# ben-watt-es/madigan

Hardware: AMD Instinct MI355X
Metric: env-steps/sec (batched) at 8192 envs × 8 assets; % HBM roofline (higher is better)
Workload: dtype f64; 1 GPU; C3: TrendOU x8 assets per env, slippage 1e-4 + 2% cost broker, DDR eta=.001 n=1, discrete actions via action_to_transaction, auto-reset; nstep=1, n_envs_per_gpu=8192, n_envs_total=8192, n_assets=8, window=0, assets_per_lane=1, schedule=trio, parallelism=env-sharded x1 (no per-step collective)

## Files before the change

### madigan_amd/csrc/mgn_diag.h

```cpp
#pragma once

#if !defined(MGN_DIAG) &&                                                                            \
    (defined(MGN_STAMPS) || defined(MGN_WALLX) || defined(MGN_ITERSTAMP) || defined(MGN_ABL_NOSTORE) ||  \
     defined(MGN_ABL_NOSTORE_ASSET) || defined(MGN_ABL_NOSTORE_ENV) || defined(MGN_ABL_DRAW) ||          \
     defined(MGN_TRIO_ABL_PRO) || defined(MGN_TRIO_ABL_G) || defined(MGN_TRIO_ABL_L) ||                  \
     defined(MGN_TRIO_ABL_F) || defined(MGN_TRIO_ABL_EPI) || defined(MGN_NST_ABL_TERM) ||                \
     defined(MGN_NST_ABL_SUM) || defined(MGN_NST_ABL_ROW) || defined(MGN_NO_GK) ||                      \
     defined(MGN_ABL_PLAIN_OFF))
#error "stamp / ablation switches belong to diagnostic builds (-DMGN_DIAG, tools/build_variant.py)"
#endif

namespace mgn {

#ifdef MGN_STAMPS
#define MGN_ST(...) __VA_ARGS__
#else
#define MGN_ST(...)
#endif
#ifdef MGN_TRIO_ABL_PRO
constexpr bool kAblPro = true;
#else
constexpr bool kAblPro = false;
#endif
#ifdef MGN_TRIO_ABL_G
// ... 39 lines not shown
#ifdef MGN_ABL_NOSTORE_ENV
constexpr bool kAblNoStoreEnv = true;
#else
constexpr bool kAblNoStoreEnv = false;
#endif
#ifdef MGN_ABL_PLAIN_OFF
constexpr bool kAblPlainOff = true;
#else
constexpr bool kAblPlainOff = false;
#endif

#ifdef MGN_STAMPS
__device__ unsigned long long g_duo_stamps[24];
__device__ unsigned long long g_trio_par[16];
#define MGN_PAR(acc, j, work, wait)                      \
  {                                                      \
    const unsigned long long w_ = (work), a_ = (wait);   \
    const bool o_ = ((j) & 1) != 0;                      \
    acc[0] += o_ ? 0 : w_;                               \
    acc[1] += o_ ? 0 : a_;                               \
    acc[2] += o_ ? w_ : 0;                               \
    acc[3] += o_ ? a_ : 0;                               \
  }
__shared__ unsigned long long s_duo_sub[8];
__device__ unsigned long long g_duo_wall[2048 * 32];
#define MGN_T(v) v = __builtin_amdgcn_s_memtime()
#define MGN_WALL(i) if ((threadIdx.x & 255) == 0 && blockIdx.x < 2048) g_duo_wall[blockIdx.x * 32 + (i)] = __builtin_amdgcn_s_memrealtime()
#elif defined(MGN_WALLX)
__device__ unsigned long long g_duo_stamps[24];
__device__ unsigned long long g_duo_wall[2048 * 32];
#define MGN_T(v)
#define MGN_WALL(i) if ((threadIdx.x & 255) == 0 && blockIdx.x < 2048) g_duo_wall[blockIdx.x * 32 + (i)] = __builtin_amdgcn_s_memrealtime()
#else
#define MGN_T(v)
#define MGN_WALL(i)
#endif
#ifdef MGN_WALLX
#define MGN_RT(v) v = __builtin_amdgcn_s_memrealtime()
#define MGN_WALLV(i, val_) if ((threadIdx.x & 255) == 0 && blockIdx.x < 2048) g_duo_wall[blockIdx.x * 32 + (i)] = (val_)
#else
#define MGN_RT(v)
#define MGN_WALLV(i, val_)
#endif

#ifdef MGN_ITERSTAMP
__device__ unsigned long long g_iter[256 * 64];
// ... 12 lines not shown
```

### madigan_amd/csrc/mgn_launch_a8t.hip

```cpp
#include "mgn_launch_impl.h"
MGN_DEFINE_UNIT(a8t)
#if defined(MGN_STAMPS) || defined(MGN_WALLX)
extern "C" int mgn_diag_stamps(unsigned long long* h) {
  if (hipMemcpyFromSymbol(h, HIP_SYMBOL(mgn::g_duo_stamps), 24 * sizeof(unsigned long long)) != hipSuccess)
    return 1;
  unsigned long long z[24] = {};
  return hipMemcpyToSymbol(HIP_SYMBOL(mgn::g_duo_stamps), z, sizeof(z)) != hipSuccess;
}
#ifdef MGN_STAMPS
extern "C" int mgn_diag_parity(unsigned long long* h) {
  if (hipMemcpyFromSymbol(h, HIP_SYMBOL(mgn::g_trio_par), 16 * sizeof(unsigned long long)) != hipSuccess)
    return 1;
  unsigned long long z[16] = {};
  return hipMemcpyToSymbol(HIP_SYMBOL(mgn::g_trio_par), z, sizeof(z)) != hipSuccess;
}
#endif
extern "C" int mgn_diag_wall(unsigned long long* h) {
  return hipMemcpyFromSymbol(h, HIP_SYMBOL(mgn::g_duo_wall), 2048 * 32 * sizeof(unsigned long long)) != hipSuccess;
}
#endif
#ifdef MGN_ITERSTAMP
extern "C" int mgn_diag_iter(unsigned long long* h) {
  if (hipMemcpyFromSymbol(h, HIP_SYMBOL(mgn::g_iter), 256 * 64 * sizeof(unsigned long long)) != hipSuccess)
    return 1;
  static unsigned long long z[256 * 64] = {};
  return hipMemcpyToSymbol(HIP_SYMBOL(mgn::g_iter), z, sizeof(z)) != hipSuccess;
}
#endif
```

### madigan_amd/csrc/mgn_math.h

```cpp
#pragma once

#include <hip/hip_runtime.h>
#include <stdint.h>

namespace mgn {

__device__ __forceinline__ double bits_to_d(uint64_t u) { return __longlong_as_double((long long)u); }
__device__ __forceinline__ uint64_t d_to_bits(double d) { return (uint64_t)__double_as_longlong(d); }

struct u4 { uint32_t x, y, z, w; };

__device__ __forceinline__ u4 philox4x32_10(uint32_t c0, uint32_t c1, uint32_t c2, uint32_t c3,
                                            uint32_t k0, uint32_t k1) {
#pragma unroll
  for (int r = 0; r < 10; ++r) {
    const uint64_t p0 = (uint64_t)0xD2511F53u * c0;
    const uint64_t p1 = (uint64_t)0xCD9E8D57u * c2;
    const uint32_t n0 = (uint32_t)(p1 >> 32) ^ c1 ^ k0;
    const uint32_t n2 = (uint32_t)(p0 >> 32) ^ c3 ^ k1;
    c0 = n0; c1 = (uint32_t)p1; c2 = n2; c3 = (uint32_t)p0;
    k0 += 0x9E3779B9u;
    k1 += 0xBB67AE85u;
  }
  return u4{c0, c1, c2, c3};
// ... 126 lines not shown
  q = __builtin_fma(__builtin_fma(-y, q, x), r, q);
  if (!fast) {
    double xs = x;
    asm volatile("" : "+v"(xs));
    q = xs / y;
  }
  return q;
}
__device__ __forceinline__ double rt_div(double a, double b) {
  if (!__builtin_amdgcn_class(b, kNormalClass)) return a / b;
  double r = __builtin_amdgcn_rcp(b);
  r = __builtin_fma(r, __builtin_fma(-b, r, 1.0), r);
  r = __builtin_fma(r, __builtin_fma(-b, r, 1.0), r);
  return a * r;
}
__device__ __forceinline__ double rt_sqrt(double x) {
  if (!__builtin_amdgcn_class(x, 1 << 8)) return sqrt(x);
  const double y = __builtin_amdgcn_rsq(x);
  double g = x * y, h = 0.5 * y;
  const double r = __builtin_fma(-g, h, 0.5);
  g = __builtin_fma(g, r, g);
  h = __builtin_fma(h, r, h);
  return __builtin_fma(__builtin_fma(-g, g, x), h, g);
}

struct Draw {
  double z, ut;
  uint32_t dbit;
};

__device__ __forceinline__ double v_log(double x) {
  const double ln2_hi = bits_to_d(0x3fe62e42fee00000ull);
  const double ln2_lo = bits_to_d(0x3dea39ef35793c76ull);
  const double Lg1 = bits_to_d(0x3FE5555555555593ull), Lg2 = bits_to_d(0x3FD999999997FA04ull),
               Lg3 = bits_to_d(0x3FD2492494229359ull), Lg4 = bits_to_d(0x3FCC71C51D8E78AFull),
               Lg5 = bits_to_d(0x3FC7466496CB03DEull), Lg6 = bits_to_d(0x3FC39A09D078C69Full),
               Lg7 = bits_to_d(0x3FC2F112DF3E5244ull);
  const uint64_t ix = d_to_bits(x);
  int32_t hx = (int32_t)(ix >> 32);
  int32_t k = ((hx >> 20) & 0x7ff) - 1023;
  hx &= 0x000fffff;
  const int32_t i = (hx + 0x95f64) & 0x100000;
  k += (i >> 20);
  const uint64_t mb = ((uint64_t)(uint32_t)(hx | (i ^ 0x3ff00000)) << 32) | (ix & 0xffffffffull);
  const double f = bits_to_d(mb) - 1.0;
  const double s = f / (2.0 + f);
// ... 81 lines not shown
__device__ __forceinline__ double normal_of(const u4& x) {
  double sn, cs;
  v_sincos2pi((double)x.z * TWO_M32, sn, cs);
  return v_radius(x) * cs;
}

__device__ __forceinline__ double log_ratio(double x) {
  const double d = x - 1.0;
  if (fabs(d) <= 0.03125) {
    const double u = x + 1.0;
    const double e = x - (u - 1.0);
    const double sh = rt_div(d, u);
    const double r = __fma_rn(-sh, u, d);
    const double sl = (r - sh * e) * 0.5;
    const double s2 = sh * sh;
    const double t =
        s2 * (0.3333333333333333 + s2 * (0.2 + s2 * (0.14285714285714285 + s2 * 0.1111111111111111)));
    const double s_2 = sh + sh;
    return s_2 + ((sl + sl) + s_2 * t);
  }
  return log(x);
}

__device__ __forceinline__ double frac_part(double x) { return copysign(x - trunc(x), x); }

__device__ __forceinline__ double log_norm(double x) { return log((x < 1e-5) ? 1e-5 : x); }

__device__ __noinline__ double det_asin(double x) {
  const double pio2_hi = bits_to_d(0x3FF921FB54442D18ull), pio2_lo = bits_to_d(0x3C91A62633145C07ull),
               pio4_hi = bits_to_d(0x3FE921FB54442D18ull);
  const double pS0 = bits_to_d(0x3FC5555555555555ull), pS1 = bits_to_d(0xBFD4D61203EB6F7Dull),
               pS2 = bits_to_d(0x3FC9C1550E884455ull), pS3 = bits_to_d(0xBFA48228B5688F3Bull),
               pS4 = bits_to_d(0x3F49EFE07501B288ull), pS5 = bits_to_d(0x3F023DE10DFDF709ull),
               qS1 = bits_to_d(0xC0033A271C8A2D4Bull), qS2 = bits_to_d(0x40002AE59C598AC8ull),
               qS3 = bits_to_d(0xBFE6066C1B8D0159ull), qS4 = bits_to_d(0x3FB3B8C5B12E9282ull);
  const uint64_t bx = d_to_bits(x);
  const int32_t hx = (int32_t)(bx >> 32);
  const int32_t ix = hx & 0x7fffffff;
  if (ix >= 0x3ff00000) {
    if (((ix - 0x3ff00000) | (int32_t)(uint32_t)bx) == 0) return x * pio2_hi + x * pio2_lo;
    return (x - x) / (x - x);
  }
  if (ix < 0x3fe00000) {
    if (ix < 0x3e400000) return x;
    const double t = x * x;
    const double p = t * (pS0 + t * (pS1 + t * (pS2 + t * (pS3 + t * (pS4 + t * pS5)))));
// ... 25 lines not shown
```

### madigan_amd/csrc/mgn_shapers.h

```cpp
#pragma once

#include <hip/hip_runtime.h>
#include <stdint.h>

#include "../../include/madigan_amd.h"
#include "mgn_math.h"
#include "mgn_params.h"
#include "mgn_reduce.h"

namespace mgn {

__device__ __forceinline__ double dsr_one(double r, double A, double B) {
  const double dA = r - A;
  const double dB = r * r - B;
  const double t = B - A * A;
  const double a = fabs(t);
  return rt_div(B * dA - (A * dB) / 2, a * rt_sqrt(a) + 1.1920928955078125e-07);
}
__device__ __forceinline__ double ddr_one(double r, double A, double B) {
  const double sB = rt_sqrt(B);
  const double h = r - A / 2;
  const bool pos = r > 0.;
  const double num = pos ? h : (B * h - (A * (r * r)) / 2);
  const double den = (pos ? sB : B * sB) + 1.1920928955078125e-07;
  return rt_div(num, den);
}
struct DdrPre {
  double hA, dpos, dneg;
};
__device__ __forceinline__ DdrPre ddr_pre(double A, double B) {
  const double sB = rt_sqrt(B);
  return DdrPre{A / 2, sB + 1.1920928955078125e-07, B * sB + 1.1920928955078125e-07};
}
__device__ __forceinline__ double ddr_one_pre(double r, double A, double B, const DdrPre& q) {
  const double h = r - q.hA;
  const bool pos = r > 0.;
  const double num = pos ? h : (B * h - (A * (r * r)) / 2);
  return rt_div(num, pos ? q.dpos : q.dneg);
}
__device__ __forceinline__ double rt_rcp(double b) {
  double r = __builtin_amdgcn_rcp(b);
  r = __builtin_fma(r, __builtin_fma(-b, r, 1.0), r);
  return __builtin_fma(r, __builtin_fma(-b, r, 1.0), r);
}
__device__ __forceinline__ double div_pre(double a, double b, double rb) {
  double q = a * rb;
  if (!__builtin_amdgcn_class(b, kNormalClass)) {
    double x = a;
    asm volatile("" : "+v"(x));
    q = x / b;
  }
  return q;
}
struct DdrPreR {
  DdrPre q;
  double rpos, rneg;
};
__device__ __forceinline__ DdrPreR ddr_pre_r(double A, double B) {
  const DdrPre q = ddr_pre(A, B);
  return DdrPreR{q, rt_rcp(q.dpos), rt_rcp(q.dneg)};
}
// ... 271 lines not shown
```

### madigan_amd/csrc/mgn_trio.h

```cpp
#pragma once

#include <hip/hip_runtime.h>
#include <stdint.h>

#include "../../include/madigan_amd.h"
#include "mgn_broker.h"
#include "mgn_consts.h"
#include "mgn_diag.h"
#include "mgn_gout.h"
#include "mgn_lane.h"
#include "mgn_math.h"
#include "mgn_params.h"
#include "mgn_reduce.h"
#include "mgn_rows.h"
#include "mgn_select.h"
#include "mgn_shapers.h"
#include "mgn_sources.h"

namespace mgn {


constexpr int kPrioG = 0, kPrioL = 2, kPrioF = 1;

constexpr int kNstU = 3;


__device__ __forceinline__ bool trio_exit(int j, int K, const int32_t& more) {
  if (j < K) return false;
  return !__builtin_amdgcn_readfirstlane(more);
}

template <int M, int S, bool ONE>
__device__ __forceinline__ bool rec_done(const double (&Lr)[M], const double (&P)[M], double cashv, double ml,
                                         double shv, double b, bool any_mc, const KParams& p, Sums& q,
                                         double& curEq) {
  double tlp[M];
#pragma unroll
  for (int m = 0; m < M; ++m) tlp[m] = Lr[m] * P[m];
  q.lp = canon<M, S, ONE>(tlp);
  q.ml = ml;
  q.sh = shv;
  q.b = b;
  curEq = (cashv + q.lp) - q.b;
  return any_mc || margin_call(q, cashv, p.mainM) || (curEq < 0.1 * p.init_cash);
}
// ... 66 lines not shown
  warm_kernargs<(int)(48 + sizeof(KParams) + sizeof(mgn_traj) + 8 + 16 + 4)>();
  MGN_IT(47, 0);
  const int in_kind = DISC ? IN_DISCRETE : in_kind_rt;
  constexpr int M = MM;
  constexpr bool TAIL = K1 && !RP && !WIN && MM == 1;
  constexpr bool GLOG = WIN && !RP;
  constexpr int NPADS = 2;
  constexpr bool NRUN = NST == 2;
  constexpr bool SBR = NRUN && TW == 64;
  static_assert(M == 1 || (M == 2 && !NST), "two slots per lane: one-step rewards");
  static_assert(!ONE || (S == 2 && M == 1), "a one-asset env on two lanes per role");
  constexpr int APAD = S * M;
  constexpr int TRIO_W = TW;
  constexpr int TRIO_BLOCK = 3 * TW;
  constexpr int EPB = TRIO_W / S;
  __shared__ TrioShared<S, TW, M> sh;
  __shared__ EnvRecs<APAD> recs[EPB];
  __shared__ mgn_asset_source s_src[APAD];
  __shared__ double s_tgt[MGN_MAX_ASSETS + 1];
  __shared__ double s_disc[NST ? MGN_MAX_NSTEP : 1];
  __shared__ double s_disc2[SBR ? MGN_MAX_NSTEP : 1];
  extern __shared__ __attribute__((aligned(16))) double s_nst[];
  constexpr bool FB = S == 8 && MM == 1 && !WIN && !NST && !RP && !ONE && !K1;
  __shared__ __attribute__((aligned(16))) double s_fqc[FB ? TW : 1], s_fqp[FB ? TW : 1], s_fqx[FB ? TW : 1],
      s_fqr[FB ? TW : 1];
  __shared__ int32_t s_fqk[FB ? TW : 1];
  const int role = threadIdx.x / TRIO_W;
  const int l = threadIdx.x % TRIO_W;
  constexpr bool GSLOT = GK < 0 && !RP && TW / S > 1 && M == 1;
  constexpr bool TAIL_EXACT = TAIL && !GSLOT;
  const int el = (GSLOT && role == 0) ? l % EPB : l / S;
  const int ls = (GSLOT && role == 0) ? l / EPB : l % S;
  const int lx = (el * S + ls) * M;
  const int env = blockIdx.x * EPB + el;
  const bool live = env < p.N;
  const int envc = live ? env : 0;
  const int A = p.A;
  Lane<M> s;
#pragma unroll
  for (int m = 0; m < M; ++m) {
    s.asset[m] = ls * M + m;
    s.valid[m] = live && ls * M + m < A;
  }
  s.rcur = 0;
  s.row = 0;
  s.pf_ok = false;
  s.fcol = (RP && p.F <= APAD) ? ls * M : -1;
  const size_t li = (size_t)envc * A + (s.valid[0] ? ls * M : 0);
  constexpr int NQ = (RP || M > 1) ? 0 : GK == MGN_SRC_TRENDOU ? 9 : GK == MGN_SRC_OU ? 3 : 0;
  constexpr bool QREG = NQ > 0;
  double qr[QREG ? NQ : 1];
  const double* const tgt_g = p.target;
#pragma unroll
  for (int m = 0; m < M; ++m) {
    s.P[m] = kAblPro ? 5.0 : ((s.valid[m] && role != 2) ? kP[li + m] : 0.);
    s.L[m] = s.mep[m] = s.Bm[m] = s.sx[m] = s.oum[m] = s.dy[m] = 0.;
    s.tlen[m] = 0;
    s.tfl[m] = 0;
  }
  uint64_t ts = 0;
  double cash = 0.;
  int act_cur[M] = {};
  const MGN_G int8_t* act_lane = vptr(act_in) + li;
  double ep_ret = 0., ep_len = 0., n_done = 0.;
  double shA = 0., shB = 0.;
  int32_t rhead = 0, rlen = 0;
  int32_t nlen = 0, nhead = 0;
  NstRun nrs{0., 0., 0., 0., 0., 0.};
  int32_t nsl = 0;
  int32_t fcnt = 0, fdone = 0;
  if (!kAblPro && role == 0) {
    constexpr bool r_sx = GK < 0 || GK == MGN_SRC_SINE || GK == MGN_SRC_SAWTOOTH || GK == MGN_SRC_TRIANGLE ||
                          GK == MGN_SRC_TRENDYOU;
    constexpr bool r_oum = GK < 0 || GK == MGN_SRC_TRENDOU || GK == MGN_SRC_TRENDYOU || GK == MGN_SRC_OUPAIR;
    constexpr bool r_trend = GK < 0 || GK == MGN_SRC_TRENDOU || GK == MGN_SRC_SIMPLETREND ||
                             GK == MGN_SRC_TRENDYOU;
#pragma unroll
    for (int m = 0; m < M; ++m) {
      if (s.valid[m]) {
        if (r_sx) s.sx[m] = p.sx[li + m];
        if (r_oum) s.oum[m] = p.oum[li + m];
        if (r_trend) {
          s.dy[m] = p.dy[li + m];
          s.tlen[m] = p.tlen[li + m];
          s.tfl[m] = p.tfl[li + m];
        }
      }
    }
    if constexpr (QREG) {
      const double* q = p.src[s.valid[0] ? ls : 0].p;
#pragma unroll
      for (int i = 0; i < NQ; ++i) qr[i] = q[i];
    }
// ... 143 lines not shown
  if (role == 0) {
    p.seed = in_vgpr(p.seed);
    p.env_offset = in_vgpr(p.env_offset);
    drain_vmem();
    MGN_IT(54, 0);
    int k = 0;
    constexpr bool SV_P = GK < 0 || !(GK == MGN_SRC_TRENDOU || GK == MGN_SRC_SIMPLETREND ||
                                      GK == MGN_SRC_TRENDYOU || GK == MGN_SRC_OUPAIR);
    constexpr bool SV_SX = GK < 0 || GK != MGN_SRC_TRENDYOU;
    constexpr bool SV_OUM = GK < 0 || !(GK == MGN_SRC_TRENDOU || GK == MGN_SRC_TRENDYOU || GK == MGN_SRC_OUPAIR);
    constexpr bool SV_TLEN = GK < 0 || !(GK == MGN_SRC_TRENDOU || GK == MGN_SRC_SIMPLETREND || GK == MGN_SRC_TRENDYOU);
    constexpr bool SV_TFL = GK < 0 || GK != MGN_SRC_SIMPLETREND;
    double svP[M] = {}, svSx[M] = {}, svOum[M] = {}, svDy[M] = {};
    int32_t svTlen[M] = {};
    uint8_t svTfl[M] = {};
    uint64_t svTs = 0;
    Lane<M> s2;
    gen_state_copy<M>(s2, s);
    uint64_t ts2 = 0;
    bool shadow = false, tail_it = false, stored = false;
    int jlast = 0;
    __builtin_amdgcn_s_setprio(kPrioG);
    MGN_ST(unsigned long long T0 = 0, T1 = 0, T2 = 0, acc0 = 0, acc1 = 0, par[4] = {0, 0, 0, 0},
           dev[4] = {0, 0, 0, 0}; int jn = 0;)
    int gpend = 0;
    RpCurM<M> rp{};
    RpNextM<M> rnx{};
    auto tick = [&]() {
      if constexpr (RP) {
        trio_replay_tick<M>(s, p, ts, rp, rnx);
      } else {
        gen_tick<M, false, false, GK, true, (M > 1)>(s, p, env, ts, QREG ? qr : nullptr);
        ts = ts + 1;
      }
    };
    auto g_store = [&]() {
#pragma unroll
      for (int m = 0; m < M; ++m) {
        const int kd = GK >= 0 ? GK : s.kind[m];
        const bool w_sx =
            kd == MGN_SRC_SINE || kd == MGN_SRC_SAWTOOTH || kd == MGN_SRC_TRIANGLE || kd == MGN_SRC_TRENDYOU;
        const bool w_oum = kd == MGN_SRC_TRENDOU || kd == MGN_SRC_TRENDYOU || kd == MGN_SRC_OUPAIR;
        const bool w_trend = kd == MGN_SRC_TRENDOU || kd == MGN_SRC_SIMPLETREND || kd == MGN_SRC_TRENDYOU;
        if (s.valid[m]) {
          const size_t i = (size_t)env * A + s.asset[m];
          p.P[i] = s.P[m];
          if (w_sx) p.sx[i] = s.sx[m];
// ... 105 lines not shown
        sh.price[cur][lx + m] = s.P[m];
        if (DISC) sh.prcp[cur][lx + m] = rcp_refined(s.P[m]);
      }
      if constexpr (GLOG) {
        if (p.ring_log != 0) {
#pragma unroll
          for (int m = 0; m < M; ++m) sh.lprice[cur][lx + m] = log_norm(s.P[m]);
        }
      }
      if (ls == 0) sh.ts[cur][el] = ts;
      if constexpr (RP) {
        if (ls == 0) {
          sh.row[cur][el] = rp.row;
          sh.dend[cur][el] = rp.dend;
        }
#pragma unroll
        for (int m = 0; m < M; ++m) sh.feat[cur][lx + m] = rp.curF[m];
      }
      if (j == 0) MGN_IT(48, 0);
      MGN_T(T1);
      __syncthreads();
      MGN_T(T2);
      MGN_IT(2 + (j < 40 ? j : 40), 0);
      MGN_ST(acc0 += T1 - T0; acc1 += T2 - T1; jn = j; MGN_PAR(par, j, T1 - T0, T2 - T1))
      jlast = j;
      if (trio_exit(j, K, sh.more[j % 3])) break;
    }
    MGN_ST(if (threadIdx.x == 0) {
      atomicAdd(&g_duo_stamps[0], acc0);
      atomicAdd(&g_duo_stamps[1], acc1);
      atomicAdd(&g_duo_stamps[8], (unsigned long long)(jn + 1));
      atomicAdd(&g_duo_stamps[10], 1ull);
      for (int i = 0; i < 4; ++i) atomicAdd(&g_trio_par[i], par[i]);
      atomicAdd(&g_trio_par[12], dev[0]);
      atomicAdd(&g_trio_par[13], dev[2]);
      atomicAdd(&g_trio_par[14], dev[1]);
      atomicAdd(&g_trio_par[15], dev[3]);
    })
    if constexpr (kAblEpi) return;
    if constexpr (TAIL) {
      if (live && shadow && !sh.reset[jlast & 1][el]) {
        gen_state_copy<M>(s, s2);
        ts = ts2;
      }
    }
    if (live && !stored) {
      g_store();
      if (RP && ls == 0) p.rcur[env] = s.rcur;
    }
    MGN_IT_DRAIN();
    MGN_IT(44, 0);
    return;
  }

  if (role == 1) {
    const uint32_t om = OMC ? OMC : traj_mask(out);
    const MGN_G double* gunits = vptr(units_in);
    const MGN_G int32_t* gaidx = vptr(aidx_in);
    p.init_cash = in_vgpr(p.init_cash);
    p.mainM = in_vgpr(p.mainM);
// ... 14 lines not shown
                 bO = (size_t)env * (A + 1);
    Sums sa = port_sums<M, S, ONE>(s.L, s.mep, s.Bm, s.P);
    drain_vmem();
    MGN_IT(51, TRIO_W);
    int k = 0;
    int lpend = 0;
    int jlast = 0;
    int lflags = 0;
    bool lstored = false;
    auto l_store = [&]() {
#pragma unroll
      for (int m = 0; m < M; ++m) {
        if (s.valid[m]) {
          const size_t i = (size_t)env * A + s.asset[m];
          p.L[i] = s.L[m];
          p.mep[i] = s.mep[m];
          p.Bm[i] = s.Bm[m];
        }
      }
      if (ls == 0) p.cash[env] = cash;
    };
    __builtin_amdgcn_s_setprio(kPrioL);
    MGN_ST(unsigned long long T0 = 0, T1 = 0, T2 = 0, acc0 = 0, acc1 = 0;
           unsigned long long Lp1 = 0, Lp2 = 0, Lp3 = 0, lacc[4] = {0, 0, 0, 0}, par[4] = {0, 0, 0, 0};)
    for (int j = 0;; ++j) {
      const int cur = j & 1, prv = cur ^ 1;
      MGN_T(T0);
      MGN_ST(Lp1 = Lp2 = Lp3 = T0;)
      if (TAIL_EXACT && K == 1 && j == 1) __builtin_amdgcn_s_setprio(kPrioG);
      const int rs_rec = sh.reset[prv][el], fl_rec = sh.rFlags[prv][el];
      double p_rec[M], r_rec[M];
#pragma unroll
      for (int m = 0; m < M; ++m) {
        p_rec[m] = sh.price[prv][lx + m];
        r_rec[m] = DISC ? sh.prcp[prv][lx + m] : 0.;
      }
      asm volatile("" ::: "memory");
      const bool rst = live && j > 0 && rs_rec != 0;
      const bool prev_step = j > 0 && (fl_rec & TR_STEP) != 0;
      const bool refill = WIN && live && (rst || lpend > 0);
      if (WIN && !rst && lpend > 0) lpend -= 1;
#pragma unroll
      for (int m = 0; m < M; ++m)
        if (j > 0 && live && s.valid[m]) s.P[m] = p_rec[m];
      if (rst) {
        if (prev_step) k -= 1;
#pragma unroll
// ... 142 lines not shown
            }
          }
          l_store();
          lstored = true;
        }
      }
      if (WIN && refill) {
#pragma unroll
        for (int m = 0; m < M; ++m) sh.rL[cur][lx + m] = s.L[m];
        if (ls == 0) {
          sh.rCash[cur][el] = cash;
          sh.rB[cur][el] = 0.;
        }
        flags = TR_REFILL;
      }
      if (ls == 0) sh.rFlags[cur][el] = flags;
      if (live && (stepping || refill || k < K || (WIN && (rst || lpend > 0)))) sh.more[j % 3] = 1;
      jlast = j;
      if (j == 0) MGN_IT(49, TRIO_W);
      MGN_T(T1);
      __syncthreads();
      MGN_T(T2);
      MGN_ST(acc0 += T1 - T0; acc1 += T2 - T1; MGN_PAR(par, j, T1 - T0, T2 - T1)
             if (Lp3 != T0) {
               lacc[0] += Lp1 - T0;
               lacc[1] += Lp2 - Lp1;
               lacc[2] += Lp3 - Lp2;
               lacc[3] += T1 - Lp3;
             })
      if (trio_exit(j, K, sh.more[j % 3])) break;
    }
    MGN_ST(if (l == 0) {
      atomicAdd(&g_duo_stamps[4], acc0);
      atomicAdd(&g_duo_stamps[5], acc1);
      for (int i = 0; i < 3; ++i) atomicAdd(&g_duo_stamps[13 + i], s_duo_sub[i]);
      atomicAdd(&g_duo_stamps[18], s_duo_sub[5]);
      atomicAdd(&g_duo_stamps[19], s_duo_sub[6]);
      atomicAdd(&g_duo_stamps[2], s_duo_sub[3]);
      atomicAdd(&g_duo_stamps[3], s_duo_sub[4]);
      atomicAdd(&g_duo_stamps[6], s_duo_sub[7]);
      for (int i = 0; i < 4; ++i) atomicAdd(&g_duo_stamps[20 + i], lacc[i]);
      for (int i = 0; i < 4; ++i) atomicAdd(&g_trio_par[4 + i], par[i]);
    })
    if constexpr (kAblEpi) return;
    if constexpr (TAIL) {
      if (live && !lstored && sh.reset[jlast & 1][el]) {
#pragma unroll
        for (int m = 0; m < M; ++m) {
          s.L[m] = 0.;
          s.mep[m] = 0.;
          s.Bm[m] = 0.;
        }
        cash = p.init_cash;
      }
    }
    if (live && !lstored) l_store();
    MGN_IT_DRAIN();
    MGN_IT(45, TRIO_W);
    return;
  }

  const uint32_t om = OMC ? OMC : traj_mask(out);
  const GTraj ov = traj_vgpr<OMC>(out);
  GState gs;
  gs.epstats = vptr(p.epstats);
// ... 104 lines not shown
      if (WIN) {
        p.rhead[env] = rhead;
        p.rlen[env] = rlen;
      }
      p.ep[(size_t)env * 2] = ep_ret;
      p.ep[(size_t)env * 2 + 1] = ep_len;
      if (D == 1) {
        p.sA[env] = g.shA;
        p.sB[env] = g.shB;
      }
    }
    if (D != 1 && s.valid[0]) {
      p.sA[(size_t)env * A + s.asset[0]] = g.shA;
      p.sB[(size_t)env * A + s.asset[0]] = g.shB;
    }
  };
  const bool fbat = FB && D == 1 && !need_ar &&
                    (p.shaper == MGN_SHAPER_NONE || p.shaper == MGN_SHAPER_DSR || p.shaper == MGN_SHAPER_DDR);
  const auto f_wave_sync = [&]() {
    __builtin_amdgcn_fence(__ATOMIC_RELEASE, "wavefront");
    __builtin_amdgcn_wave_barrier();
    __builtin_amdgcn_fence(__ATOMIC_ACQUIRE, "wavefront");
  };
  const auto f_flush = [&]() {
    if constexpr (FB) {
      f_wave_sync();
      const bool mine = ls < fcnt;
      const double curEq = mine ? s_fqc[l] : 1., prevEq = mine ? s_fqp[l] : 1.;
      const int k = s_fqk[l];
      const double ratio = curEq / prevEq;
      const double clampv = (in_kind == IN_SINGLE) ? 0.01 : 0.3;
      const double reward = log_ratio((ratio < clampv) ? clampv : ratio);
      double x = mine ? s_fqx[l] : 0.;
      asm volatile("" : "+v"(x));
      const double port0 = x / curEq;
      s_fqr[l] = reward;
      f_wave_sync();
      double r[S];
#pragma unroll
      for (int i = 0; i < S; ++i) r[i] = s_fqr[el * S + i];
      double Ai = g.shA, Bi = g.shB;
      int last = -1;
      double st_ret = 0., st_len = 0.;
#pragma unroll
      for (int i = 0; i < S; ++i) {
        if (ls == i) {
          Ai = g.shA;
          Bi = g.shB;
        }
        if (i < fcnt) {
          const double ri = r[i];
          if (p.shaper == MGN_SHAPER_DDR) {
            double m = ri < 0. ? ri : 0.;
            if (ri != ri) m = ri;
            g.shA += p.eta * (ri - g.shA);
            g.shB += p.eta * (m * m - g.shB);
          } else if (p.shaper == MGN_SHAPER_DSR) {
            g.shA += p.eta * (ri - g.shA);
            g.shB += p.eta * (ri * ri - g.shB);
          }
          ep_ret += ri;
          ep_len += 1;
          if ((fdone >> i) & 1) {
            st_ret = ep_ret;
            st_len = ep_len;
            n_done = n_done + 1;
            last = i;
            ep_ret = 0;
            ep_len = 0;
          }
        }
      }
      if (last >= 0 && ls == 0) {
        MGN_G double* st = gs.epstats + (size_t)env * 4;
        st[0] = st_ret;
        st[1] = st_len;
        st[2] = s_fqc[el * S + last];
        st[3] = n_done;
      }
      if (!kAblNoStoreEnv && mine) {
        double shaped_s = reward;
        if (p.shaper == MGN_SHAPER_DDR)
          shaped_s = clip1((0.0 + 1.0 * ddr_one_pre(reward, Ai, Bi, ddr_pre(Ai, Bi))) / 1);
        else if (p.shaper == MGN_SHAPER_DSR)
          shaped_s = clip1((0.0 + 1.0 * dsr_one(reward, Ai, Bi)) / 1);
        const size_t ie = kidx(k, sN, (size_t)env);
        if (om & O_OPT) ost(ov.obs_port + kidx(k, sNA1, bO), port0);
        if (om & O_REW) ost(ov.reward + ie, reward);
        if (om & O_SHP) ost(ov.shaped + ie, shaped_s);
      }
      fcnt = 0;
      fdone = 0;
    }
  };
  drain_vmem();
  __builtin_amdgcn_s_setprio(kPrioF);
  MGN_ST(unsigned long long T0 = 0, T1 = 0, T2 = 0, acc0 = 0, acc1 = 0, Tf1 = 0, Tf2 = 0, facc[3] = {0, 0, 0},
         par[4] = {0, 0, 0, 0};)
  for (int j = 0;; ++j) {
    const int cur = j & 1, prv = cur ^ 1;
    MGN_T(T0);
    MGN_ST(Tf1 = Tf2 = 0;)
    int rst_out = 0;
    bool tail_rst = false;
    const int flags = j > 0 ? sh.rFlags[prv][el] : 0;
    const int rsv = j > 0 ? sh.reset[prv][el] : 0;
    const int krec = sh.rK[prv][el];
    double Lrec[M], Prec[M];
#pragma unroll
    for (int m = 0; m < M; ++m) {
      Lrec[m] = sh.rL[prv][lx + m];
      Prec[m] = sh.price[prv][lx + m];
    }
    const double cashrec = sh.rCash[prv][el], prevrec = sh.rPrevEq[prv][el];
    asm volatile("" ::: "memory");
    if (!kAblF && live && (flags & TR_STEP) && !rsv) {
      const int k = krec;
      NstPre npre{};
      double nst_w = 0., nst_r0 = 0., nst_w2 = 0., nst_rt0 = 0.;
      if constexpr (NRUN) {
        const int n = p.nstep;
// ... 13 lines not shown
        }
        nst_w = s_disc[nlen];
        nst_r0 = ring[nhead];
        if (SBR && p.shaper == MGN_SHAPER_SORTINO_B) {
          nst_w2 = s_disc2[nlen];
          nst_rt0 = ring[nst_pad(n, S) + nhead];
        }
        npre = nrun_pre(p.shaper, nrs, nlen + 1, g.shA, g.shB);
      }
      Lane<M> f = s;
#pragma unroll
      for (int m = 0; m < M; ++m) {
        f.L[m] = Lrec[m];
        f.P[m] = Prec[m];
      }
      const double cashv = cashrec;
      const double prevEq = prevrec;
      Sums q;
      double curEq;
      const bool done = rec_done<M, S, ONE>(f.L, f.P, cashv, sh.rMl[prv][el], sh.rSh[prv][el], sh.rB[prv][el],
                                            (flags & TR_ANYMC) != 0, p, q, curEq);
      if (j == 1) MGN_IT(55, 2 * TRIO_W);
      if (FB && fbat) {
        if (ls == fcnt) {
          const int e = el * S + fcnt;
          s_fqc[e] = curEq;
          s_fqp[e] = prevEq;
          s_fqx[e] = cashv - q.b;
          s_fqk[e] = k;
        }
        fdone |= (done ? 1 : 0) << fcnt;
        fcnt += 1;
        MGN_ST(Tf1 = Tf2 = __builtin_amdgcn_s_memtime();)
        if (!kAblNoStoreAsset && f.valid[0]) {
          if (om & O_OPR) ost(ov.obs_price + kidx(k, sNF, bP), f.P[0]);
          if (om & O_OPT) {
            double x = f.L[0] * f.P[0];
            asm volatile("" : "+v"(x));
            ost(ov.obs_port + (kidx(k, sNA1, bO) + 1 + f.asset[0]), x / curEq);
          }
        }
        if (!kAblNoStoreEnv && ls == 0) {
          const size_t ie = kidx(k, sN, (size_t)env);
          if (om & O_DONE) ost(ov.done + ie, (uint8_t)(done ? 1 : 0));
          if (om & O_MC) {
            const Sums qa{sh.rLpA[prv][el], q.ml, q.sh, q.b};
            const bool mcall = (flags & TR_MCALL) && margin_call(qa, cashv, p.mainM);
            ost(ov.margin_call + ie, (uint8_t)(mcall ? 1 : 0));
          }
          if (om & O_DEND) ost(ov.data_end + ie, (uint8_t)0u);
          if (om & O_NSH) ost(ov.n_shaped + ie, (uint8_t)1);
          if (om & O_TS) ost(ov.timestamp + ie, (uint64_t)sh.ts[prv][el]);
        }
        if (done && p.auto_reset) rst_out = 1;
// ... 210 lines not shown
          rhead = p.W - 1;
        }
      }
      ep_ret += reward;
      ep_len += 1;
      if (done) {
        if (ls == 0) {
          MGN_G double* st = gs.epstats + (size_t)env * 4;
          st[0] = ep_ret;
          st[1] = ep_len;
          st[2] = curEq;
          n_done = n_done + 1;
          st[3] = n_done;
        }
        ep_ret = 0;
        ep_len = 0;
        if (p.auto_reset) {
          rst_out = 1;
          tail_rst = TAIL && K == 1;
        }
      }
      }
    }
    if (FB && fbat && j > 0 && (j & (S - 1)) == 0) f_flush();
    if (WIN && live && (flags & TR_REFILL)) {
      double Pf[M], Lf[M], tlp[M], pa[M];
#pragma unroll
      for (int m = 0; m < M; ++m) {
        Pf[m] = sh.price[prv][lx + m];
        Lf[m] = sh.rL[prv][lx + m];
        tlp[m] = Lf[m] * Pf[m];
      }
      const double cashf = sh.rCash[prv][el], bf = sh.rB[prv][el];
      const double eq = (cashf + canon<M, S, ONE>(tlp)) - bf;
#pragma unroll
      for (int m = 0; m < M; ++m) pa[m] = (Lf[m] * Pf[m]) / eq;
      push_row(Pf, pa, (cashf - bf) / eq, (uint64_t)sh.ts[prv][el], klast, prv);
    }
    if constexpr (TAIL_EXACT) {
      if (K == 1 && j == 1 && live) {
        f_store();
        fstored = true;
      }
    }
    if (ls == 0) sh.reset[cur][el] = rst_out;
    if (rst_out && !tail_rst) sh.more[j % 3] = 1;
    if (j == 1) MGN_IT(50, 2 * TRIO_W);
    MGN_T(T1);
    __syncthreads();
    MGN_T(T2);
    MGN_ST(acc0 += T1 - T0; acc1 += T2 - T1; MGN_PAR(par, j, T1 - T0, T2 - T1)
           if (Tf2) {
             facc[0] += Tf1 - T0;
             facc[1] += Tf2 - Tf1;
             facc[2] += T1 - Tf2;
           })
    if (trio_exit(j, K, sh.more[j % 3])) break;
  }
  MGN_ST(if (l == 0) {
    atomicAdd(&g_duo_stamps[16], acc0);
    atomicAdd(&g_duo_stamps[17], acc1);
    atomicAdd(&g_duo_stamps[9], facc[0]);
    atomicAdd(&g_duo_stamps[11], facc[1]);
    atomicAdd(&g_duo_stamps[12], facc[2]);
    for (int i = 0; i < 4; ++i) atomicAdd(&g_trio_par[8 + i], par[i]);
  })
  if constexpr (kAblEpi) return;
  if (FB && fbat && __builtin_amdgcn_ballot_w64(fcnt > 0) != 0) f_flush();
  if (!live) return;
  if constexpr (NST != 0) {
    const double* ring = s_nst + (size_t)el * NPADS * nst_pad(p.nstep, S);
    for (int i = ls; i < p.nstep; i += S) p.nring[(size_t)env * p.nstep + i] = ring[i];
    if (ls == 0) {
      p.nlen[env] = nlen;
      p.nhead[env] = nhead;
    }
  }
  if (!fstored) f_store();
  MGN_IT_DRAIN();
  MGN_IT(46, 2 * TRIO_W);
}

}
```

Before: 4.918 billion env-steps/s.

## Parameterize deferred flush queue depth and batch reward/shaper math across queued entries

New measurement: 4.958 billion env-steps/s, median of 3. Within noise of the previous version (+0.8%).

```diff
diff --git a/madigan_amd/csrc/mgn_diag.h b/madigan_amd/csrc/mgn_diag.h
--- a/madigan_amd/csrc/mgn_diag.h
+++ b/madigan_amd/csrc/mgn_diag.h
@@ -85,6 +85,16 @@
     acc[2] += o_ ? w_ : 0;                               \
     acc[3] += o_ ? a_ : 0;                               \
   }
+__device__ unsigned long long g_trio_flush[16];
+#define MGN_FLP(acc, j, depth, work, wait)               \
+  {                                                      \
+    const unsigned long long w_ = (work), a_ = (wait);   \
+    const bool o_ = (j) > 0 && (j) % (depth) == 0;       \
+    acc[0] += o_ ? 0 : w_;                               \
+    acc[1] += o_ ? 0 : a_;                               \
+    acc[2] += o_ ? w_ : 0;                               \
+    acc[3] += o_ ? a_ : 0;                               \
+  }
 __shared__ unsigned long long s_duo_sub[8];
 __device__ unsigned long long g_duo_wall[2048 * 32];
 #define MGN_T(v) v = __builtin_amdgcn_s_memtime()
diff --git a/madigan_amd/csrc/mgn_launch_a8t.hip b/madigan_amd/csrc/mgn_launch_a8t.hip
--- a/madigan_amd/csrc/mgn_launch_a8t.hip
+++ b/madigan_amd/csrc/mgn_launch_a8t.hip
@@ -14,6 +14,13 @@
   unsigned long long z[16] = {};
   return hipMemcpyToSymbol(HIP_SYMBOL(mgn::g_trio_par), z, sizeof(z)) != hipSuccess;
 }
+extern "C" int mgn_diag_flush(unsigned long long* h) {
+  if (hipMemcpyFromSymbol(h, HIP_SYMBOL(mgn::g_trio_flush), 16 * sizeof(unsigned long long)) != hipSuccess)
+    return 1;
+  h[16] = (unsigned long long)mgn::kFqDepth;
+  unsigned long long z[16] = {};
+  return hipMemcpyToSymbol(HIP_SYMBOL(mgn::g_trio_flush), z, sizeof(z)) != hipSuccess;
+}
 #endif
 extern "C" int mgn_diag_wall(unsigned long long* h) {
   return hipMemcpyFromSymbol(h, HIP_SYMBOL(mgn::g_duo_wall), 2048 * 32 * sizeof(unsigned long long)) != hipSuccess;
diff --git a/madigan_amd/csrc/mgn_math.h b/madigan_amd/csrc/mgn_math.h
--- a/madigan_amd/csrc/mgn_math.h
+++ b/madigan_amd/csrc/mgn_math.h
@@ -172,6 +172,43 @@
   g = __builtin_fma(g, r, g);
   h = __builtin_fma(h, r, h);
   return __builtin_fma(__builtin_fma(-g, g, x), h, g);
+}
+
+template <int W>
+__device__ __forceinline__ void rt_div_n(const double (&a)[W], const double (&b)[W], double (&out)[W]) {
+  bool slow = false;
+#pragma unroll
+  for (int i = 0; i < W; ++i) {
+    slow |= !__builtin_amdgcn_class(b[i], kNormalClass);
+    double r = __builtin_amdgcn_rcp(b[i]);
+    r = __builtin_fma(r, __builtin_fma(-b[i], r, 1.0), r);
+    r = __builtin_fma(r, __builtin_fma(-b[i], r, 1.0), r);
+    out[i] = a[i] * r;
+  }
+  if (__builtin_amdgcn_ballot_w64(slow) != 0) {
+#pragma unroll
+    for (int i = 0; i < W; ++i)
+      if (!__builtin_amdgcn_class(b[i], kNormalClass)) out[i] = a[i] / b[i];
+  }
+}
+template <int W>
+__device__ __forceinline__ void rt_sqrt_n(const double (&x)[W], double (&out)[W]) {
+  bool slow = false;
+#pragma unroll
+  for (int i = 0; i < W; ++i) {
+    slow |= !__builtin_amdgcn_class(x[i], 1 << 8);
+    const double y = __builtin_amdgcn_rsq(x[i]);
+    double g = x[i] * y, h = 0.5 * y;
+    const double r = __builtin_fma(-g, h, 0.5);
+    g = __builtin_fma(g, r, g);
+    h = __builtin_fma(h, r, h);
+    out[i] = __builtin_fma(__builtin_fma(-g, g, x[i]), h, g);
+  }
+  if (__builtin_amdgcn_ballot_w64(slow) != 0) {
+#pragma unroll
+    for (int i = 0; i < W; ++i)
+      if (!__builtin_amdgcn_class(x[i], 1 << 8)) out[i] = sqrt(x[i]);
+  }
 }
 
 struct Draw {
@@ -299,6 +336,39 @@
   return log(x);
 }
 
+template <int W>
+__device__ __forceinline__ void log_ratio_n(const double (&x)[W], double (&out)[W]) {
+  uint32_t pend = 0;
+#pragma unroll
+  for (int i = 0; i < W; ++i) {
+    const double d = x[i] - 1.0;
+    pend |= (fabs(d) <= 0.03125 ? 0u : 1u) << i;
+    const double u = x[i] + 1.0;
+    const double e = x[i] - (u - 1.0);
+    double rc = __builtin_amdgcn_rcp(u);
+    rc = __builtin_fma(rc, __builtin_fma(-u, rc, 1.0), rc);
+    rc = __builtin_fma(rc, __builtin_fma(-u, rc, 1.0), rc);
+    const double sh = d * rc;
+    const double r = __fma_rn(-sh, u, d);
+    const double sl = (r - sh * e) * 0.5;
+    const double s2 = sh * sh;
+    const double t =
+        s2 * (0.3333333333333333 + s2 * (0.2 + s2 * (0.14285714285714285 + s2 * 0.1111111111111111)));
+    const double s_2 = sh + sh;
+    out[i] = s_2 + ((sl + sl) + s_2 * t);
+  }
+  while (pend) {
+    const int c = __builtin_ctz(pend);
+    pend &= pend - 1;
+    double xs = x[0];
+#pragma unroll
+    for (int i = 1; i < W; ++i) xs = (c == i) ? x[i] : xs;
+    const double y = log(xs);
+#pragma unroll
+    for (int i = 0; i < W; ++i) out[i] = (c == i) ? y : out[i];
+  }
+}
+
 __device__ __forceinline__ double frac_part(double x) { return copysign(x - trunc(x), x); }
 
 __device__ __forceinline__ double log_norm(double x) { return log((x < 1e-5) ? 1e-5 : x); }
diff --git a/madigan_amd/csrc/mgn_shapers.h b/madigan_amd/csrc/mgn_shapers.h
--- a/madigan_amd/csrc/mgn_shapers.h
+++ b/madigan_amd/csrc/mgn_shapers.h
@@ -37,6 +37,38 @@
   const bool pos = r > 0.;
   const double num = pos ? h : (B * h - (A * (r * r)) / 2);
   return rt_div(num, pos ? q.dpos : q.dneg);
+}
+template <int W>
+__device__ __forceinline__ void ddr_one_n(const double (&r)[W], const double (&A)[W], const double (&B)[W],
+                                          double (&out)[W]) {
+  double sB[W], num[W], den[W];
+  rt_sqrt_n<W>(B, sB);
+#pragma unroll
+  for (int i = 0; i < W; ++i) {
+    const double hA = A[i] / 2, dpos = sB[i] + 1.1920928955078125e-07,
+                 dneg = B[i] * sB[i] + 1.1920928955078125e-07;
+    const double h = r[i] - hA;
+    const bool pos = r[i] > 0.;
+    num[i] = pos ? h : (B[i] * h - (A[i] * (r[i] * r[i])) / 2);
+    den[i] = pos ? dpos : dneg;
+  }
+  rt_div_n<W>(num, den, out);
+}
+template <int W>
+__device__ __forceinline__ void dsr_one_n(const double (&r)[W], const double (&A)[W], const double (&B)[W],
+                                          double (&out)[W]) {
+  double a[W], sa[W], num[W], den[W];
+#pragma unroll
+  for (int i = 0; i < W; ++i) a[i] = fabs(B[i] - A[i] * A[i]);
+  rt_sqrt_n<W>(a, sa);
+#pragma unroll
+  for (int i = 0; i < W; ++i) {
+    const double dA = r[i] - A[i];
+    const double dB = r[i] * r[i] - B[i];
+    num[i] = B[i] * dA - (A[i] * dB) / 2;
+    den[i] = a[i] * sa[i] + 1.1920928955078125e-07;
+  }
+  rt_div_n<W>(num, den, out);
 }
 __device__ __forceinline__ double rt_rcp(double b) {
   double r = __builtin_amdgcn_rcp(b);
diff --git a/madigan_amd/csrc/mgn_trio.h b/madigan_amd/csrc/mgn_trio.h
--- a/madigan_amd/csrc/mgn_trio.h
+++ b/madigan_amd/csrc/mgn_trio.h
@@ -21,6 +21,20 @@
 
 
 constexpr int kPrioG = 0, kPrioL = 2, kPrioF = 1;
+
+#ifndef MGN_FQ
+#define MGN_FQ 1
+#endif
+#ifndef MGN_FQW
+#define MGN_FQW MGN_FQ
+#endif
+#ifndef MGN_FQ_PRIO
+#define MGN_FQ_PRIO 0
+#endif
+constexpr int kFq = MGN_FQ, kFqW = MGN_FQW, kFqDepth = 8 * kFq, kFqPrio = MGN_FQ_PRIO;
+struct FlushInLoop { static constexpr bool value = false; };
+struct FlushClosing { static constexpr bool value = true; };
+static_assert(kFq >= 1 && kFq <= 4 && kFqW >= 1 && kFq % kFqW == 0, "1..4 entries per lane, in whole groups");
 
 constexpr int kNstU = 3;
 
@@ -133,9 +147,9 @@
   __shared__ double s_disc2[SBR ? MGN_MAX_NSTEP : 1];
   extern __shared__ __attribute__((aligned(16))) double s_nst[];
   constexpr bool FB = S == 8 && MM == 1 && !WIN && !NST && !RP && !ONE && !K1;
-  __shared__ __attribute__((aligned(16))) double s_fqc[FB ? TW : 1], s_fqp[FB ? TW : 1], s_fqx[FB ? TW : 1],
-      s_fqr[FB ? TW : 1];
-  __shared__ int32_t s_fqk[FB ? TW : 1];
+  constexpr int FQ = FB ? kFq : 1, FQN = FB ? kFq * TW : 1;
+  __shared__ __attribute__((aligned(16))) double s_fqc[FQN], s_fqp[FQN], s_fqx[FQN], s_fqr[FQN];
+  __shared__ int32_t s_fqk[FQN];
   const int role = threadIdx.x / TRIO_W;
   const int l = threadIdx.x % TRIO_W;
   constexpr bool GSLOT = GK < 0 && !RP && TW / S > 1 && M == 1;
@@ -179,7 +193,8 @@
   int32_t nlen = 0, nhead = 0;
   NstRun nrs{0., 0., 0., 0., 0., 0.};
   int32_t nsl = 0;
-  int32_t fcnt = 0, fdone = 0;
+  int32_t fcnt = 0;
+  uint32_t fdone = 0;
   if (!kAblPro && role == 0) {
     constexpr bool r_sx = GK < 0 || GK == MGN_SRC_SINE || GK == MGN_SRC_SAWTOOTH || GK == MGN_SRC_TRIANGLE ||
                           GK == MGN_SRC_TRENDYOU;
@@ -369,7 +384,7 @@
     int jlast = 0;
     __builtin_amdgcn_s_setprio(kPrioG);
     MGN_ST(unsigned long long T0 = 0, T1 = 0, T2 = 0, acc0 = 0, acc1 = 0, par[4] = {0, 0, 0, 0},
-           dev[4] = {0, 0, 0, 0}; int jn = 0;)
+           dev[4] = {0, 0, 0, 0}, flp[4] = {0, 0, 0, 0}, fln[4] = {0, 0, 0, 0}; int jn = 0;)
     int gpend = 0;
     RpCurM<M> rp{};
     RpNextM<M> rnx{};
@@ -521,7 +536,8 @@
       __syncthreads();
       MGN_T(T2);
       MGN_IT(2 + (j < 40 ? j : 40), 0);
-      MGN_ST(acc0 += T1 - T0; acc1 += T2 - T1; jn = j; MGN_PAR(par, j, T1 - T0, T2 - T1))
+      MGN_ST(acc0 += T1 - T0; acc1 += T2 - T1; jn = j; MGN_PAR(par, j, T1 - T0, T2 - T1)
+             MGN_FLP(flp, j, kFqDepth, T1 - T0, T2 - T1) MGN_FLP(fln, j, kFqDepth, 1, 0))
       jlast = j;
       if (trio_exit(j, K, sh.more[j % 3])) break;
     }
@@ -535,6 +551,9 @@
       atomicAdd(&g_trio_par[13], dev[2]);
       atomicAdd(&g_trio_par[14], dev[1]);
       atomicAdd(&g_trio_par[15], dev[3]);
+      for (int i = 0; i < 4; ++i) atomicAdd(&g_trio_flush[i], flp[i]);
+      atomicAdd(&g_trio_flush[12], fln[0]);
+      atomicAdd(&g_trio_flush[13], fln[2]);
     })
     if constexpr (kAblEpi) return;
     if constexpr (TAIL) {
@@ -595,7 +614,8 @@
     };
     __builtin_amdgcn_s_setprio(kPrioL);
     MGN_ST(unsigned long long T0 = 0, T1 = 0, T2 = 0, acc0 = 0, acc1 = 0;
-           unsigned long long Lp1 = 0, Lp2 = 0, Lp3 = 0, lacc[4] = {0, 0, 0, 0}, par[4] = {0, 0, 0, 0};)
+           unsigned long long Lp1 = 0, Lp2 = 0, Lp3 = 0, lacc[4] = {0, 0, 0, 0}, par[4] = {0, 0, 0, 0},
+           flp[4] = {0, 0, 0, 0};)
     for (int j = 0;; ++j) {
       const int cur = j & 1, prv = cur ^ 1;
       MGN_T(T0);
@@ -784,6 +804,7 @@
       __syncthreads();
       MGN_T(T2);
       MGN_ST(acc0 += T1 - T0; acc1 += T2 - T1; MGN_PAR(par, j, T1 - T0, T2 - T1)
+             MGN_FLP(flp, j, kFqDepth, T1 - T0, T2 - T1)
              if (Lp3 != T0) {
                lacc[0] += Lp1 - T0;
                lacc[1] += Lp2 - Lp1;
@@ -803,6 +824,7 @@
       atomicAdd(&g_duo_stamps[6], s_duo_sub[7]);
       for (int i = 0; i < 4; ++i) atomicAdd(&g_duo_stamps[20 + i], lacc[i]);
       for (int i = 0; i < 4; ++i) atomicAdd(&g_trio_par[4 + i], par[i]);
+      for (int i = 0; i < 4; ++i) atomicAdd(&g_trio_flush[4 + i], flp[i]);
     })
     if constexpr (kAblEpi) return;
     if constexpr (TAIL) {
@@ -953,81 +975,140 @@
     __builtin_amdgcn_wave_barrier();
     __builtin_amdgcn_fence(__ATOMIC_ACQUIRE, "wavefront");
   };
-  const auto f_flush = [&]() {
+  const auto f_flush = [&](auto closing) {
     if constexpr (FB) {
+      constexpr bool CL = decltype(closing)::value;
+      constexpr int W = CL ? 1 : kFqW;
+      if (!CL && kFqPrio > 0) __builtin_amdgcn_s_setprio(kFqPrio);
       f_wave_sync();
-      const bool mine = ls < fcnt;
-      const double curEq = mine ? s_fqc[l] : 1., prevEq = mine ? s_fqp[l] : 1.;
-      const int k = s_fqk[l];
-      const double ratio = curEq / prevEq;
       const double clampv = (in_kind == IN_SINGLE) ? 0.01 : 0.3;
-      const double reward = log_ratio((ratio < clampv) ? clampv : ratio);
-      double x = mine ? s_fqx[l] : 0.;
-      asm volatile("" : "+v"(x));
-      const double port0 = x / curEq;
-      s_fqr[l] = reward;
+      bool mine[FQ], use[FQ];
+#pragma unroll
+      for (int q = 0; q < FQ; ++q) {
+        mine[q] = q * S + ls < fcnt;
+        use[q] = !CL || q == 0 || __builtin_amdgcn_ballot_w64(fcnt > q * S) != 0;
+      }
+#pragma unroll
+      for (int q0 = 0; q0 < FQ; q0 += W) {
+        if (use[q0]) {
+          double ce[W], pe[W], xx[W], ra[W], rw[W], port0[W];
+          int kq[W];
+#pragma unroll
+          for (int w = 0; w < W; ++w) {
+            const int e = (q0 + w) * TW + l;
+            double c = s_fqc[e], pv = s_fqp[e], xv = s_fqx[e];
+            asm volatile("" : "+v"(c), "+v"(pv), "+v"(xv));
+            ce[w] = mine[q0 + w] ? c : 1.;
+            pe[w] = mine[q0 + w] ? pv : 1.;
+            xx[w] = mine[q0 + w] ? xv : 0.;
+            kq[w] = s_fqk[e];
+          }
+#pragma unroll
+          for (int w = 0; w < W; ++w) {
+            const double ratio = ce[w] / pe[w];
+            ra[w] = (ratio < clampv) ? clampv : ratio;
+          }
+          log_ratio_n<W>(ra, rw);
+#pragma unroll
+          for (int w = 0; w < W; ++w) {
+            double x = xx[w];
+            asm("" : "+v"(x));
+            port0[w] = x / ce[w];
+            s_fqr[(q0 + w) * TW + l] = rw[w];
+          }
+          if (!kAblNoStoreEnv) {
+#pragma unroll
+            for (int w = 0; w < W; ++w) {
+              if (mine[q0 + w]) {
+                if (om & O_OPT) ost(ov.obs_port + kidx(kq[w], sNA1, bO), port0[w]);
+                if (om & O_REW) ost(ov.reward + kidx(kq[w], sN, (size_t)env), rw[w]);
+              }
+            }
+          }
+        }
+      }
       f_wave_sync();
-      double r[S];
-#pragma unroll
-      for (int i = 0; i < S; ++i) r[i] = s_fqr[el * S + i];
-      double Ai = g.shA, Bi = g.shB;
       int last = -1;
       double st_ret = 0., st_len = 0.;
-#pragma unroll
-      for (int i = 0; i < S; ++i) {
-        if (ls == i) {
-          Ai = g.shA;
-          Bi = g.shB;
-        }
-        if (i < fcnt) {
+      const bool ddr = p.shaper == MGN_SHAPER_DDR, upd = ddr || p.shaper == MGN_SHAPER_DSR;
+#pragma nounroll
+      for (int q = 0; q < FQ; ++q) {
+        if (CL && q > 0 && __builtin_amdgcn_ballot_w64(fcnt > q * S) == 0) break;
+        double r[S];
+#pragma unroll
+        for (int i = 0; i < S; ++i) r[i] = s_fqr[q * TW + el * S + i];
+        double Aq = g.shA, Bq = g.shB;
+#pragma unroll
+        for (int i = 0; i < S; ++i) {
+          const int e = q * S + i;
+          if (ls == i) {
+            Aq = g.shA;
+            Bq = g.shB;
+          }
+          const bool act = e < fcnt;
           const double ri = r[i];
-          if (p.shaper == MGN_SHAPER_DDR) {
-            double m = ri < 0. ? ri : 0.;
-            if (ri != ri) m = ri;
-            g.shA += p.eta * (ri - g.shA);
-            g.shB += p.eta * (m * m - g.shB);
-          } else if (p.shaper == MGN_SHAPER_DSR) {
-            g.shA += p.eta * (ri - g.shA);
-            g.shB += p.eta * (ri * ri - g.shB);
-          }
-          ep_ret += ri;
-          ep_len += 1;
-          if ((fdone >> i) & 1) {
-            st_ret = ep_ret;
-            st_len = ep_len;
-            n_done = n_done + 1;
-            last = i;
-            ep_ret = 0;
-            ep_len = 0;
-          }
-        }
+          double m = ri < 0. ? ri : 0.;
+          m = (ri != ri) ? ri : m;
+          const double sq = ddr ? m * m : ri * ri;
+          const double a1 = g.shA + p.eta * (ri - g.shA);
+          const double b1 = g.shB + p.eta * (sq - g.shB);
+          g.shA = (act && upd) ? a1 : g.shA;
+          g.shB = (act && upd) ? b1 : g.shB;
+          const double er = ep_ret + ri, en = ep_len + 1;
+          const bool dn = act && ((fdone >> e) & 1) != 0;
+          st_ret = dn ? er : st_ret;
+          st_len = dn ? en : st_len;
+          n_done = dn ? n_done + 1 : n_done;
+          last = dn ? e : last;
+          ep_ret = dn ? 0. : (act ? er : ep_ret);
+          ep_len = dn ? 0. : (act ? en : ep_len);
+        }
+        s_fqp[q * TW + l] = Aq;
+        s_fqx[q * TW + l] = Bq;
       }
       if (last >= 0 && ls == 0) {
         MGN_G double* st = gs.epstats + (size_t)env * 4;
         st[0] = st_ret;
         st[1] = st_len;
-        st[2] = s_fqc[el * S + last];
+        st[2] = s_fqc[(last / S) * TW + el * S + (last & (S - 1))];
         st[3] = n_done;
       }
-      if (!kAblNoStoreEnv && mine) {
-        double shaped_s = reward;
-        if (p.shaper == MGN_SHAPER_DDR)
-          shaped_s = clip1((0.0 + 1.0 * ddr_one_pre(reward, Ai, Bi, ddr_pre(Ai, Bi))) / 1);
-        else if (p.shaper == MGN_SHAPER_DSR)
-          shaped_s = clip1((0.0 + 1.0 * dsr_one(reward, Ai, Bi)) / 1);
-        const size_t ie = kidx(k, sN, (size_t)env);
-        if (om & O_OPT) ost(ov.obs_port + kidx(k, sNA1, bO), port0);
-        if (om & O_REW) ost(ov.reward + ie, reward);
-        if (om & O_SHP) ost(ov.shaped + ie, shaped_s);
+      if (!kAblNoStoreEnv && (om & O_SHP)) {
+#pragma unroll
+        for (int q0 = 0; q0 < FQ; q0 += W) {
+          if (use[q0]) {
+            double rw[W], Ai[W], Bi[W], shaped[W];
+            int kq[W];
+#pragma unroll
+            for (int w = 0; w < W; ++w) {
+              rw[w] = s_fqr[(q0 + w) * TW + l];
+              Ai[w] = s_fqp[(q0 + w) * TW + l];
+              Bi[w] = s_fqx[(q0 + w) * TW + l];
+              kq[w] = s_fqk[(q0 + w) * TW + l];
+              shaped[w] = rw[w];
+            }
+            if (ddr) {
+              ddr_one_n<W>(rw, Ai, Bi, shaped);
+            } else if (upd) {
+              dsr_one_n<W>(rw, Ai, Bi, shaped);
+            }
+#pragma unroll
+            for (int w = 0; w < W; ++w) shaped[w] = upd ? clip1((0.0 + 1.0 * shaped[w]) / 1) : rw[w];
+#pragma unroll
+            for (int w = 0; w < W; ++w)
+              if (mine[q0 + w]) ost(ov.shaped + kidx(kq[w], sN, (size_t)env), shaped[w]);
+          }
+        }
       }
       fcnt = 0;
       fdone = 0;
+      if (!CL && kFqPrio > 0) __builtin_amdgcn_s_setprio(kPrioF);
     }
   };
   drain_vmem();
   __builtin_amdgcn_s_setprio(kPrioF);
   MGN_ST(unsigned long long T0 = 0, T1 = 0, T2 = 0, acc0 = 0, acc1 = 0, Tf1 = 0, Tf2 = 0, facc[3] = {0, 0, 0},
-         par[4] = {0, 0, 0, 0};)
+         par[4] = {0, 0, 0, 0}, flp[4] = {0, 0, 0, 0};)
   for (int j = 0;; ++j) {
     const int cur = j & 1, prv = cur ^ 1;
     MGN_T(T0);
@@ -1087,14 +1168,14 @@
                                             (flags & TR_ANYMC) != 0, p, q, curEq);
       if (j == 1) MGN_IT(55, 2 * TRIO_W);
       if (FB && fbat) {
-        if (ls == fcnt) {
-          const int e = el * S + fcnt;
+        if (ls == (fcnt & (S - 1))) {
+          const int e = (fcnt / S) * TW + l;
           s_fqc[e] = curEq;
           s_fqp[e] = prevEq;
           s_fqx[e] = cashv - q.b;
           s_fqk[e] = k;
         }
-        fdone |= (done ? 1 : 0) << fcnt;
+        fdone |= (done ? 1u : 0u) << fcnt;
         fcnt += 1;
         MGN_ST(Tf1 = Tf2 = __builtin_amdgcn_s_memtime();)
         if (!kAblNoStoreAsset && f.valid[0]) {
@@ -1351,7 +1432,7 @@
       }
       }
     }
-    if (FB && fbat && j > 0 && (j & (S - 1)) == 0) f_flush();
+    if (FB && fbat && j > 0 && j % kFqDepth == 0) f_flush(FlushInLoop{});
     if (WIN && live && (flags & TR_REFILL)) {
       double Pf[M], Lf[M], tlp[M], pa[M];
 #pragma unroll
@@ -1379,6 +1460,7 @@
     __syncthreads();
     MGN_T(T2);
     MGN_ST(acc0 += T1 - T0; acc1 += T2 - T1; MGN_PAR(par, j, T1 - T0, T2 - T1)
+           MGN_FLP(flp, j, kFqDepth, T1 - T0, T2 - T1)
            if (Tf2) {
              facc[0] += Tf1 - T0;
              facc[1] += Tf2 - Tf1;
@@ -1393,9 +1475,10 @@
     atomicAdd(&g_duo_stamps[11], facc[1]);
     atomicAdd(&g_duo_stamps[12], facc[2]);
     for (int i = 0; i < 4; ++i) atomicAdd(&g_trio_par[8 + i], par[i]);
+    for (int i = 0; i < 4; ++i) atomicAdd(&g_trio_flush[8 + i], flp[i]);
   })
   if constexpr (kAblEpi) return;
-  if (FB && fbat && __builtin_amdgcn_ballot_w64(fcnt > 0) != 0) f_flush();
+  if (FB && fbat && __builtin_amdgcn_ballot_w64(fcnt > 0) != 0) f_flush(FlushClosing{});
   if (!live) return;
   if constexpr (NST != 0) {
     const double* ring = s_nst + (size_t)el * NPADS * nst_pad(p.nstep, S);
```
